# AdamQLMeng/PPNet

Hardware: AMD Instinct MI355X
Metric: edage_pp_map_path_instances_per_sec (higher is better)
Workload: dtype f64

## Files before the change

include/ppnet_hip.h:

```cpp
#ifndef PPNET_HIP_H
#define PPNET_HIP_H

#include <stdint.h>

#ifdef __cplusplus
extern "C" {
#endif

#define PPN_OK             0
#define PPN_E_INVALID     -1
#define PPN_E_HIP         -2
#define PPN_E_UNSUPPORTED -3

#define PPN_SEGS            10
#define PPN_POLY             5
#define PPN_PATH_POINTS   1000
#define PPN_BOUNDARY_POINTS 1100
#define PPN_DRAWS_PER_SEG 1002
#define PPN_DRAWS_PER_PATH (1 + PPN_SEGS * PPN_DRAWS_PER_SEG)
#define PPN_MAX_HULL        64
#define PPN_MAX_ISLES       16
#define PPN_MAX_POCKET      64
#define PPN_POCKET_TRY_CAP 256
#define PPN_PLACE_TRY_CAP 4096
// ... 304 lines not shown
                    const uint32_t* params , void* img_out ,
                    uint8_t* label_out , int B, int H, int W, int Ho, int Wo,
                    const float* mean3, const float* std3, int seg_pad_val, int dtype , void* stream);
int ppn_seg_labels_2class(const void* logits, uint8_t* labels, int32_t B, int32_t h, int32_t w, int32_t Ho, int32_t Wo,
                          int32_t dtype, void* stream);
int ppn_bias_act_nhwc(void* x, const void* bias, int64_t n, int32_t C, float negative_slope, int32_t dtype, void* stream);

int ppn_conv3x3_c1_nhwc(const void* x, const float* w, const float* bias, void* y, int32_t B, int32_t H, int32_t W,
                        int32_t Cout, float negative_slope, int32_t dtype, void* stream);
int ppn_conv3x3_to1_nhwc(const void* x, const float* w, float bias, void* y, int32_t B, int32_t H, int32_t W, int32_t Cin,
                         int32_t dtype, void* stream);

int ppn_conv3x3_mfma_bf16(const void* x, const void* w, const float* bias, void* y, int32_t B, int32_t H, int32_t W, int32_t Cin,
                          int32_t Cout, int32_t stride, int32_t relu, void* stream);
int32_t ppn_conv3x3_relu_classify2_slots(int32_t Cout);
int ppn_conv3x3_relu_classify2_bf16(const void* x, const void* w, const float* bias, const float* w2, float* logits, float* partial, int32_t B,
                                    int32_t H, int32_t W, int32_t Cin, int32_t Cout, void* stream);
int ppn_gennet_conv_s2_bf16(const void* x, const void* w, const float* bias, void* y, int32_t B, int32_t H, int32_t W, float negative_slope,
                            int32_t transposed, void* stream);
int ppn_gennet_dec_final_bf16(const void* x, const void* w, const float* bias, float negative_slope, const float* w_final, float bias_final, void* y,
                              int32_t B, int32_t H, int32_t W, void* stream);
int ppn_gennet_first_enc_bf16(const void* x1, const void* w1, const float* b1, const void* wk2, const float* bias2, void* y, int32_t B, int32_t H, int32_t W,
                              float slope1, float slope2, void* stream);
#define PPN_GENNET_BLOCK_PARAMS 7224
int ppn_gennet_trunk_bf16(const void* x, void* y, const float* params, int32_t B, int32_t N, int32_t n_blocks, void* stream);
int ppn_assemble_paths(const double* wp, const int32_t* wp_n, const uint8_t* ok, const double* init, const double* end, double rate, int32_t n,
                       int32_t max_wp, double* full, int32_t* counts, void* stream);
int ppn_plan_collision(const double* waypoints, const int32_t* counts, const void* obstacles, int32_t obstacles_f64, const int32_t* n_obstacles,
                       int32_t B, int32_t M, int32_t S, float clearance, float bound, uint8_t* collision, void* stream);
int ppn_heatmap_u8(const void* y, uint8_t* out, int32_t B, int32_t n, int32_t dtype, void* stream);
int ppn_tokenizer_conv1_codes_bf16(const uint8_t* grid, const void* lut, void* out, int32_t B, int32_t H, int32_t W, void* stream);
int ppn_tokenizer_codes_bf16(const uint8_t* grid, const void* lut, const void* w2p, const float* vec, void* tokens, int32_t B, int32_t H, int32_t W,
                             float eps, void* stream);
int ppn_nat128_ln_qkv_bf16(const void* s, const float* offset, const void* ln_w, const void* ln_b, const void* w, const void* bias, void* qkv,
                           int64_t tokens, float eps, void* stream);
int ppn_nat128_ln_mlp_bf16(void* s, const float* offset, const void* ln_w, const void* ln_b, const void* w1, const void* b1, const void* w2,
                           int64_t tokens, float eps, void* stream);
int ppn_nat128_ln_mlp_add_bf16(void* s, const float* offset, const void* ln_w, const void* ln_b, const void* w1, const void* b1, const void* w2,
                               const float* final_add, int64_t tokens, float eps, void* stream);
int ppn_nat128_proj_add_bf16(void* s, const void* a, const void* w, int64_t tokens, void* stream);

int ppn_gemm_bf16(const void* a, const void* w, const float* bias, void* c, int64_t M, int32_t N, int32_t K, int32_t epilogue,
                  int32_t persistent_blocks, void* stream);

int32_t ppn_nat_gemm_partials(int32_t C);

// ... 21 lines not shown
```

ppnet_amd/_lib.py:

```python
import ctypes as C
import os

_HERE = os.path.dirname(os.path.abspath(__file__))
LIB_PATH = os.environ.get("PPNET_HIP_LIB") or os.path.join(_HERE, "libppnet_hip.so")

PPN_OK = 0
PPN_E_UNSUPPORTED = -3
SEGS = 10
PATH_POINTS = 1000
BOUNDARY_POINTS = 1100
DRAWS_PER_SEG = 1002
DRAWS_PER_PATH = 1 + SEGS * DRAWS_PER_SEG
MAX_HULL = 64
MAX_ISLES = 16
MAX_POCKET = 64
POCKET_TRY_CAP = 256
PLACE_TRY_CAP = 4096
MAX_WAYPOINTS = 2048
GRID_OBST, GRID_FREE, GRID_MARK = 0, 255, 128
FLAG_POCKET_CAP, FLAG_PLACE_CAP, FLAG_EMPTY_ISLE, FLAG_HULL_CAP, FLAG_ISLE_CAP, FLAG_POCKET_FULL = 1, 2, 4, 8, 16, 32
FLAG_CORRIDOR_PASS = 64
FLAG_POCKET_DRAWS = 128

_p = C.c_void_p
# ... 19 lines not shown

ABI_VERSION = 111

EXPORTS = ("ppn_version", "ppn_error_string", "ppn_last_hip_error", "ppn_polyfit_table", "ppn_edage_paths",
           "ppn_edage_paths_ex", "ppn_edage_paths_ex2", "ppn_edage_maps", "ppn_edage_maps_place", "ppn_edage_maps_raster",
           "ppn_label_masks", "ppn_boundary_check", "ppn_boundary_check_ex",
           "ppn_obstacle_filter", "ppn_paint_markers", "ppn_disc_raster", "ppn_collision_segments", "ppn_collision_segments_bound",
           "ppn_extract_paths", "ppn_resize_bilinear_u8", "ppn_philox_doubles", "ppn_na2d_fwd", "ppn_na2d_fwd_padded", "ppn_na2d_fwd_vpad", "ppn_swin_wmsa_fwd", "ppn_swin_wmsa_bwd", "ppn_swin_wmsa_bwd_workspace", "ppn_mhsa_fwd", "ppn_mhsa_bwd", "ppn_mhsa_bwd_workspace", "ppn_na2d_bwd", "ppn_na2d_bwd_workspace", "ppn_na2d_bwd_vpad", "ppn_na2d_bwd_vpad_workspace", "ppn_residual_layernorm", "ppn_residual_layernorm_padded", "ppn_layernorm_offset", "ppn_upsample2x_nhwc", "ppn_resize_concat4_nhwc", "ppn_resize_concat_nhwc", "ppn_adaptive_pools_nhwc", "ppn_upsample2x_add_nhwc", "ppn_upsample2x_nhwc_bias", "ppn_upsample2x_concat_nhwc", "ppn_bias_act_nhwc", "ppn_seg_labels_2class", "ppn_grid_to_image", "ppn_conv3x3_c1_nhwc", "ppn_conv3x3_to1_nhwc",
           "ppn_conv3x3_mfma_bf16", "ppn_conv3x3_relu_classify2_bf16", "ppn_conv3x3_relu_classify2_slots", "ppn_gemm_bf16", "ppn_nat_gemm_bf16", "ppn_nat_gemm_partials", "ppn_row_stats_bf16", "ppn_nat_mlp_supported", "ppn_nat_mlp_pack_bf16", "ppn_nat_mlp_bf16", "ppn_gennet_conv_s2_bf16", "ppn_gennet_trunk_bf16",
           "ppn_assemble_paths", "ppn_plan_collision", "ppn_gennet_first_enc_bf16", "ppn_gennet_dec_final_bf16", "ppn_heatmap_u8", "ppn_tokenizer_conv1_codes_bf16", "ppn_tokenizer_codes_bf16", "ppn_nat128_ln_qkv_bf16", "ppn_nat128_ln_mlp_bf16", "ppn_nat128_ln_mlp_add_bf16", "ppn_nat128_proj_add_bf16",
           "ppn_resize_ce_workspace", "ppn_resize_ce_fwd", "ppn_resize_ce_bwd", "ppn_seg_eval",
           "ppn_augment_params", "ppn_augment_codes", "ppn_augment_rgb",
           "ppn_ohem_ce_workspace", "ppn_ohem_ce_fwd", "ppn_ohem_ce_bwd",
           "ppn_resize_dice_workspace", "ppn_resize_dice_fwd", "ppn_resize_dice_bwd",
           "ppn_upsample2x_nhwc_bwd", "ppn_upsample2x_concat_nhwc_bwd", "ppn_resize_concat_nhwc_bwd",
           "ppn_residual_layernorm_train_fwd", "ppn_residual_layernorm_bwd_workspace", "ppn_residual_layernorm_bwd",
           "ppn_patch_merge_ln_fwd", "ppn_patch_merge_ln_bwd_workspace", "ppn_patch_merge_ln_bwd", "ppn_patch_merge_ln_rows",
           "ppn_patch_merge_ln_max_blocks", "ppn_seg_tta",
           "ppn_gennet_stem_train_workspace", "ppn_gennet_stem_train_fwd", "ppn_gennet_stem_train_bwd", "ppn_gennet_stem_train_tile",
           "ppn_gennet_stem_train_max_blocks",
           "ppn_gennet_tail_train_workspace", "ppn_gennet_tail_train_fwd", "ppn_gennet_tail_train_bwd", "ppn_gennet_tail_train_tile",
           "ppn_gennet_tail_train_max_blocks",
           "ppn_gennet_s2_tile", "ppn_gennet_s2_max_blocks", "ppn_gennet_s2_wgrad_workspace", "ppn_gennet_s2_down", "ppn_gennet_s2_up",
           "ppn_gennet_s2_wgrad", "ppn_wmsa_fwd")


def _load():
    if not os.path.exists(LIB_PATH):
        raise ImportError(
            f"{LIB_PATH} is missing: the HIP extension is the only implementation of this package "
            f"(no CPU fallback). Build it with `python -c 'import __graft_entry__ as g; g.build()'` "
            f"or `make -C ppnet_amd/csrc`.")
    lib = C.CDLL(LIB_PATH)
    lib.ppn_version.restype = C.c_int
    if lib.ppn_version() != ABI_VERSION:
        raise ImportError(
            f"{LIB_PATH} reports ABI version {lib.ppn_version()}, these bindings are written against {ABI_VERSION} "
            f"(include/ppnet_hip.h: PPN_ABI_VERSION): argument lists differ, rebuild with `make -C ppnet_amd/csrc`.")
    lib.ppn_error_string.restype = C.c_char_p
    lib.ppn_error_string.argtypes = [C.c_int]
    lib.ppn_last_hip_error.restype = C.c_int
    lib.ppn_polyfit_table.argtypes = [_p]
    lib.ppn_edage_paths.argtypes = [C.c_int32, C.c_uint64, C.c_int32, C.c_double, C.c_double, C.c_uint64,
                                    _p, _p, C.c_int32, C.POINTER(PathsStruct), _p]
    lib.ppn_edage_paths_ex.argtypes = [C.c_int32, C.c_uint64, C.c_int32, C.c_double, C.c_double, C.c_uint64,
                                       _p, _p, C.c_int32, _p, C.POINTER(PathsStruct), _p]
    lib.ppn_edage_paths_ex2.argtypes = [C.c_int32, C.c_uint64, C.c_int32, C.c_double, C.c_double, C.c_uint64,
# ... 75 lines not shown
    lib.ppn_gennet_tail_train_bwd.argtypes = [_p] * 12 + [C.c_int] * 4 + [C.c_float, C.c_int, _p]
    lib.ppn_gennet_tail_train_tile.argtypes = []
    lib.ppn_gennet_tail_train_max_blocks.argtypes = []
    lib.ppn_gennet_s2_tile.argtypes = []
    lib.ppn_gennet_s2_max_blocks.argtypes = []
    lib.ppn_gennet_s2_wgrad_workspace.argtypes = [C.c_int] * 3
    lib.ppn_gennet_s2_wgrad_workspace.restype = C.c_int64
    lib.ppn_gennet_s2_down.argtypes = [_p] * 4 + [C.c_int] * 5 + [_p]
    lib.ppn_gennet_s2_up.argtypes = [_p] * 4 + [C.c_int] * 5 + [_p]
    lib.ppn_gennet_s2_wgrad.argtypes = [_p] * 6 + [C.c_int] * 5 + [_p]
    lib.ppn_grid_to_image.argtypes = [_p, _p, C.c_int64, C.POINTER(C.c_float), C.POINTER(C.c_float), C.c_int32, _p]
    lib.ppn_seg_labels_2class.argtypes = [_p, _p, C.c_int32, C.c_int32, C.c_int32, C.c_int32, C.c_int32, C.c_int32, _p]
    lib.ppn_bias_act_nhwc.argtypes = [_p, _p, C.c_int64, C.c_int32, C.c_float, C.c_int32, _p]
    lib.ppn_conv3x3_c1_nhwc.argtypes = [_p, _p, _p, _p, C.c_int32, C.c_int32, C.c_int32, C.c_int32, C.c_float, C.c_int32, _p]
    lib.ppn_conv3x3_to1_nhwc.argtypes = [_p, _p, C.c_float, _p, C.c_int32, C.c_int32, C.c_int32, C.c_int32, C.c_int32, _p]
    lib.ppn_conv3x3_mfma_bf16.argtypes = [_p, _p, _p, _p, C.c_int32, C.c_int32, C.c_int32, C.c_int32, C.c_int32, C.c_int32, C.c_int32, _p]
    lib.ppn_conv3x3_relu_classify2_bf16.argtypes = [_p, _p, _p, _p, _p, _p, C.c_int32, C.c_int32, C.c_int32, C.c_int32, C.c_int32, _p]
    lib.ppn_conv3x3_relu_classify2_slots.argtypes = [C.c_int32]
    lib.ppn_gennet_conv_s2_bf16.argtypes = [_p, _p, _p, _p, C.c_int32, C.c_int32, C.c_int32, C.c_float, C.c_int32, _p]
    lib.ppn_gennet_trunk_bf16.argtypes = [_p, _p, _p, C.c_int32, C.c_int32, C.c_int32, _p]
    lib.ppn_assemble_paths.argtypes = [_p, _p, _p, _p, _p, C.c_double, C.c_int32, C.c_int32, _p, _p, _p]
    lib.ppn_plan_collision.argtypes = [_p, _p, _p, C.c_int32, _p, C.c_int32, C.c_int32, C.c_int32, C.c_float, C.c_float, _p, _p]
    lib.ppn_gennet_first_enc_bf16.argtypes = [_p, _p, _p, _p, _p, _p, C.c_int32, C.c_int32, C.c_int32, C.c_float, C.c_float, _p]
    lib.ppn_gennet_dec_final_bf16.argtypes = [_p, _p, _p, C.c_float, _p, C.c_float, _p, C.c_int32, C.c_int32, C.c_int32, _p]
    lib.ppn_heatmap_u8.argtypes = [_p, _p, C.c_int32, C.c_int32, C.c_int32, _p]
    lib.ppn_tokenizer_conv1_codes_bf16.argtypes = [_p, _p, _p, C.c_int32, C.c_int32, C.c_int32, _p]
    lib.ppn_tokenizer_codes_bf16.argtypes = [_p, _p, _p, _p, _p, C.c_int32, C.c_int32, C.c_int32, C.c_float, _p]
    lib.ppn_nat128_ln_qkv_bf16.argtypes = [_p, _p, _p, _p, _p, _p, _p, C.c_int64, C.c_float, _p]
    lib.ppn_nat128_ln_mlp_bf16.argtypes = [_p, _p, _p, _p, _p, _p, _p, C.c_int64, C.c_float, _p]
    lib.ppn_nat128_ln_mlp_add_bf16.argtypes = [_p, _p, _p, _p, _p, _p, _p, _p, C.c_int64, C.c_float, _p]
    lib.ppn_nat128_proj_add_bf16.argtypes = [_p, _p, _p, C.c_int64, _p]
    lib.ppn_gemm_bf16.argtypes = [_p, _p, _p, _p, C.c_int64, C.c_int32, C.c_int32, C.c_int32, C.c_int32, _p]
    lib.ppn_nat_gemm_bf16.argtypes = [_p, _p, _p, _p, _p, C.c_int32, _p, _p, C.c_int64, C.c_int32, C.c_int32, C.c_int32, C.c_float, _p]
    lib.ppn_row_stats_bf16.argtypes = [_p, C.c_int64, C.c_int32, _p, _p]
    lib.ppn_nat_gemm_partials.argtypes = [C.c_int32]
    lib.ppn_nat_mlp_supported.argtypes = [C.c_int64, C.c_int32, C.c_int32]
    lib.ppn_nat_mlp_pack_bf16.argtypes = [_p, _p, _p, C.c_int32, C.c_int32, _p]
    lib.ppn_nat_mlp_bf16.argtypes = [_p, _p, _p, _p, _p, C.c_int64, C.c_int32, C.c_int32, C.c_float, _p]
    lib.ppn_resize_ce_workspace.argtypes = [C.c_int] * 3
    lib.ppn_resize_ce_workspace.restype = C.c_int64
    lib.ppn_resize_ce_fwd.argtypes = [_p, _p, _p, _p, _p, _p, C.c_int64] + [C.c_int] * 9 + [_p]
    lib.ppn_resize_ce_bwd.argtypes = [_p, _p, _p, _p, _p] + [C.c_int] * 9 + [_p]
    lib.ppn_seg_eval.argtypes = [_p, _p, _p, _p] + [C.c_int] * 9 + [_p]
    lib.ppn_seg_tta.argtypes = [C.POINTER(TtaAug), C.c_int, _p, _p] + [C.c_int] * 5 + [_p]
    lib.ppn_ohem_ce_workspace.argtypes = [C.c_int] * 3
    lib.ppn_ohem_ce_workspace.restype = C.c_int64
# ... 37 lines not shown
```

ppnet_amd/csrc/capi.hip:

```cpp
#include <hip/hip_runtime.h>
#include <math.h>
#include <mutex>
#include <stdlib.h>
#include <string.h>
#include <vector>

#include <cstdlib>
#include "ppn_kernels.h"

namespace {

thread_local int g_last_hip = 0;

inline int hip_fail(hipError_t e) {
    g_last_hip = (int)e;
    return PPN_E_HIP;
}
#define PPN_HIP(call) do { hipError_t e_ = (call); if (e_ != hipSuccess) return hip_fail(e_); } while (0)

inline bool bad_R(int R) { return R < 32 || R > 512 || (R % 32) != 0; }

void build_polyfit_table(double* out) {
    const int N = PPN_PATH_POINTS, M = 5;
    std::vector<long double> q((size_t)M * N);
// ... 1132 lines not shown
    const int e = ppn::conv3x3_mfma_launch(x, w, bias, nullptr, B, H, W, Cin, Cout, 1, 1, w2, logits, partial, (hipStream_t)stream);
    if (e != 0) return hip_fail((hipError_t)e);
    return PPN_OK;
}

int ppn_gennet_conv_s2_bf16(const void* x, const void* w, const float* bias, void* y, int32_t B, int32_t H, int32_t W, float negative_slope,
                            int32_t transposed, void* stream) {
    if (!x || !w || !bias || !y || B <= 0 || H <= 0 || W <= 0 || (!transposed && ((H | W) & 1))) return PPN_E_INVALID;
    if ((long long)B * H * W * 4 >= (1LL << 31)) return PPN_E_UNSUPPORTED;
    const int e = transposed ? ppn::gennet_dec_conv_launch(x, w, bias, y, B, H, W, negative_slope, (hipStream_t)stream)
                             : ppn::gennet_enc_conv_launch(x, w, bias, y, B, H, W, negative_slope, (hipStream_t)stream);
    if (e != 0) return hip_fail((hipError_t)e);
    return PPN_OK;
}

int ppn_gennet_first_enc_bf16(const void* x1, const void* w1, const float* b1, const void* wk2, const float* bias2, void* y, int32_t B, int32_t H, int32_t W,
                              float slope1, float slope2, void* stream) {
    if (!x1 || !w1 || !b1 || !wk2 || !bias2 || !y || B <= 0 || H <= 0 || W <= 0 || ((H | W) & 1)) return PPN_E_INVALID;
    const int e = ppn::gennet_first_enc_launch(x1, w1, b1, wk2, bias2, y, B, H, W, slope1, slope2, (hipStream_t)stream);
    if (e != 0) return hip_fail((hipError_t)e);
    return PPN_OK;
}

int ppn_gennet_dec_final_bf16(const void* x, const void* w, const float* bias, float negative_slope, const float* w_final, float bias_final, void* y,
                              int32_t B, int32_t H, int32_t W, void* stream) {
    if (!x || !w || !bias || !w_final || !y || B <= 0 || H <= 0 || W <= 0) return PPN_E_INVALID;
    if ((long long)B * H * W * 4 * 24 >= (1LL << 32)) return PPN_E_UNSUPPORTED;
    const int e = ppn::gennet_dec_final_launch(x, w, bias, negative_slope, w_final, bias_final, y, B, H, W, (hipStream_t)stream);
    if (e != 0) return hip_fail((hipError_t)e);
    return PPN_OK;
}

int ppn_gennet_trunk_bf16(const void* x, void* y, const float* params, int32_t B, int32_t N, int32_t n_blocks, void* stream) {
    if (!x || !y || !params || B <= 0 || N <= 0 || N > 1024 || (N % 8) != 0 || n_blocks <= 0) return PPN_E_INVALID;
    const int e = ppn::gennet_trunk_launch(x, y, params, B, N, n_blocks, (hipStream_t)stream);
    if (e != 0) return hip_fail((hipError_t)e);
    return PPN_OK;
}

int ppn_assemble_paths(const double* wp, const int32_t* wp_n, const uint8_t* ok, const double* init, const double* end, double rate, int32_t n,
                       int32_t max_wp, double* full, int32_t* counts, void* stream) {
    if (!wp || !wp_n || !ok || !init || !end || !full || !counts || n <= 0 || max_wp <= 0) return PPN_E_INVALID;
    const int e = ppn::assemble_paths_launch(wp, wp_n, ok, init, end, rate, n, max_wp, full, counts, (hipStream_t)stream);
    if (e != 0) return hip_fail((hipError_t)e);
    return PPN_OK;
}
// ... 155 lines not shown
```

ppnet_amd/csrc/gennet_conv.hip:

```cpp
#include <hip/hip_runtime.h>
#include "ppn_device.h"
#include "ppn_kernels.h"

namespace ppn {

namespace {
typedef __attribute__((ext_vector_type(8))) __bf16 bf16x8;
typedef __attribute__((ext_vector_type(4))) __bf16 bf16x4;
typedef __attribute__((ext_vector_type(4))) float f32x4;

__device__ __forceinline__ bf16x8 ld8(const __bf16* p) { return *reinterpret_cast<const bf16x8*>(p); }
__device__ __forceinline__ bf16x8 zero8() { return bf16x8{0, 0, 0, 0, 0, 0, 0, 0}; }

__device__ __forceinline__ void store4(__bf16* dst, const f32x4 v, const float4 b, float slope) {
    float o[4] = {v[0] + b.x, v[1] + b.y, v[2] + b.z, v[3] + b.w};
#pragma unroll
    for (int r = 0; r < 4; ++r) o[r] = o[r] > 0.f ? o[r] : o[r] * slope;
    *reinterpret_cast<bf16x4*>(dst) = bf16x4{(__bf16)o[0], (__bf16)o[1], (__bf16)o[2], (__bf16)o[3]};
}
__device__ __forceinline__ void store8(__bf16* dst, const f32x4 a0, const f32x4 a1, const float4 b0, const float4 b1, float slope) {
    float o[8] = {a0[0] + b0.x, a0[1] + b0.y, a0[2] + b0.z, a0[3] + b0.w, a1[0] + b1.x, a1[1] + b1.y, a1[2] + b1.z, a1[3] + b1.w};
#pragma unroll
    for (int r = 0; r < 8; ++r) o[r] = o[r] > 0.f ? o[r] : o[r] * slope;
    *reinterpret_cast<bf16x8*>(dst) = bf16x8{(__bf16)o[0], (__bf16)o[1], (__bf16)o[2], (__bf16)o[3], (__bf16)o[4], (__bf16)o[5], (__bf16)o[6], (__bf16)o[7]};
// ... 245 lines not shown
            const u32x4_ fw = {odd ? (w8 | 0x3F800000u) : e0, odd ? 0u : e1, odd ? 0u : e2, odd ? 0u : e3};
            const bf16x8 bw = __builtin_bit_cast(bf16x8, fw);
            f32x4 y0 = __builtin_amdgcn_mfma_f32_16x16x32_bf16(wa1[0], bw, f32x4{0.f, 0.f, 0.f, 0.f}, 0, 0, 0);
            f32x4 y1 = __builtin_amdgcn_mfma_f32_16x16x32_bf16(wa1[1], bw, f32x4{0.f, 0.f, 0.f, 0.f}, 0, 0, 0);
            const int py = 2 * oy + ty - 1, px = 2 * ox + tx - 1;
            const bool inside = py >= 0 && py < H && px >= 0 && px < W;
            float v[8] = {y0[0], y0[1], y0[2], y0[3], y1[0], y1[1], y1[2], y1[3]};
#pragma unroll
            for (int e = 0; e < 8; ++e) v[e] = fmaxf(v[e], v[e] * slope1);
            u32x4_ fv = {pack_bf16x2(v[0], v[1]), pack_bf16x2(v[2], v[3]), pack_bf16x2(v[4], v[5]), pack_bf16x2(v[6], v[7])};
            if (!inside) fv = u32x4_{0u, 0u, 0u, 0u};
            const bf16x8 fb = __builtin_bit_cast(bf16x8, fv);
            a0 = __builtin_amdgcn_mfma_f32_16x16x32_bf16(wa2[0][t], fb, a0, 0, 0, 0);
            a1 = __builtin_amdgcn_mfma_f32_16x16x32_bf16(wa2[1][t], fb, a1, 0, 0, 0);
        }
        if (live) {
            __bf16* dst = y + (size_t)pix * GC;
            store4(dst + 4 * g, a0, d0, slope2);
            if (g < 2) store4(dst + 16 + 4 * g, a1, d1, slope2);
        }
    }
}

int gennet_first_enc_launch(const void* x1, const void* w1, const float* b1, const void* wk2, const float* bias2, void* y, int B, int H, int W, float slope1,
                            float slope2, hipStream_t stream) {
    const long long total = (long long)B * (H / 2) * (W / 2);
    if ((long long)B * H * W >= (1LL << 31)) return (int)hipErrorInvalidValue;
    long long blocks = (total + 63) / 64;
    if (blocks > 256 * 12) blocks = 256 * 12;
    hipLaunchKernelGGL(gennet_first_enc_kernel, dim3((unsigned)blocks), dim3(256), 0, stream, (const __bf16*)x1, (const __bf16*)w1, b1,
                       (const __bf16*)wk2, bias2, (__bf16*)y, B, H, W, slope1, slope2);
    return (int)hipGetLastError();
}

int gennet_enc_conv_launch(const void* x, const void* wk, const float* bias, void* y, int B, int H, int W, float slope, hipStream_t stream) {
    const long long total = (long long)B * (H / 2) * (W / 2);
    long long blocks = (total + 16 * GROUPS * 4 - 1) / (16 * GROUPS * 4);
    if (blocks > 256 * 16) blocks = 256 * 16;
    hipLaunchKernelGGL(gennet_enc_conv_kernel, dim3((unsigned)blocks), dim3(256), 0, stream, (const __bf16*)x, (const __bf16*)wk, bias,
                       (__bf16*)y, B, H, W, slope);
    return (int)hipGetLastError();
}

int gennet_dec_final_launch(const void* x, const void* wt, const float* bias, float slope, const float* w1, float bias1, void* y, int B, int H, int W,
                            hipStream_t stream) {
    const long long tiles = (long long)B * ((2 * H + DF_H - 1) / DF_H) * ((2 * W + DF_W - 1) / DF_W);
// ... 20 lines not shown
```

ppnet_amd/csrc/ppn_kernels.h:

```cpp
#pragma once
#include <hip/hip_runtime.h>
#include <stdint.h>
#include <atomic>
#include "../../include/ppnet_hip.h"

#ifndef PPN_PATHS_THREADS
#define PPN_PATHS_THREADS 256
#endif

namespace ppn {

constexpr int PPN_MAX_DEVICES = 64;
inline int current_device() {
    int d = 0;
    return (hipGetDevice(&d) == hipSuccess && d >= 0 && d < PPN_MAX_DEVICES) ? d : -1;
}
struct DeviceOnce { std::atomic<int> done[PPN_MAX_DEVICES]; };
struct DeviceBuffer { std::atomic<void*> p[PPN_MAX_DEVICES]; };
inline int dynamic_lds_once(DeviceOnce& o, const void* fn, int bytes) {
    const int d = current_device();
    if (d < 0) return (int)hipErrorInvalidDevice;
    if (o.done[d].load(std::memory_order_acquire)) return 0;
    const hipError_t e = hipFuncSetAttribute(fn, hipFuncAttributeMaxDynamicSharedMemorySize, bytes);
    if (e != hipSuccess) return (int)e;
// ... 199 lines not shown
                       int label_dtype, hipStream_t stream);
int resize_dice_pixels();
int resize_dice_threads();
int resize_dice_max_classes();
long long resize_dice_workspace_bytes(int B, int C, int H, int W);
int resize_dice_fwd_launch(const void* logit, const void* label, const float* class_weight, void* workspace, float* lse, double* sums, float* loss,
                           int64_t* correct, int B, int C, int h, int w, int H, int W, int ignore_index, float smooth, int logit_dtype,
                           int label_dtype, hipStream_t stream);
int resize_dice_bwd_launch(const void* logit, const void* label, const float* lse, const double* sums, const float* class_weight,
                           const float* grad_out, void* workspace, void* dlogit, int B, int C, int h, int w, int H, int W, int ignore_index,
                           float smooth, int logit_dtype, int label_dtype, hipStream_t stream);
int augment_threads();
int augment_pixels();
int augment_params_launch(uint64_t seed, uint64_t first_instance, int B, double flip_ratio, double brightness_delta, double contrast_lo,
                          double contrast_hi, double saturation_lo, double saturation_hi, int hue_delta, uint32_t* params, hipStream_t stream);
int augment_launch(int rgb, const uint8_t* in, const uint8_t* label_in, const uint32_t* params, void* img, uint8_t* label_out, int B, int H, int W,
                   int Ho, int Wo, const float* mean, const float* stdv, int seg_pad_val, int dtype, hipStream_t stream);
int na2d_dense7_launch(const void* qkv, const void* pad_kv, const float* rpb, void* out, int B, int H, int W, int Hr, int Wr, int heads, int dil,
                       float scale, hipStream_t stream);
int gennet_dec_final_launch(const void* x, const void* wt, const float* bias, float slope, const float* w1, float bias1, void* y, int B, int H, int W,
                            hipStream_t stream);
int gennet_first_enc_launch(const void* x1, const void* w1, const float* b1, const void* wk2, const float* bias2, void* y, int B, int H, int W, float slope1,
                            float slope2, hipStream_t stream);
int heatmap_u8_launch(const void* y, uint8_t* out, int B, int n, int dtype, hipStream_t stream);
int tokenizer_fused_launch(const uint8_t* grid, const void* lut, const void* w2p, const float* vec, void* out, int B, int H, int W, float eps,
                           hipStream_t stream);
int tokenizer_codes_launch(const uint8_t* grid, const void* lut, void* out, int B, int H, int W, hipStream_t stream);
int nat128_ln_qkv_launch(const void* s, const float* off, const void* lnw, const void* lnb, const void* w, const void* bias, void* qkv, long long tokens,
                         float eps, hipStream_t stream);
int nat128_ln_mlp_launch(void* s, const float* off, const void* lnw, const void* lnb, const void* w1, const void* b1, const void* w2, const float* add,
                         long long tokens, float eps, hipStream_t stream);
int nat128_proj_add_launch(void* s, const void* a, const void* w, long long tokens, hipStream_t stream);
int gennet_trunk_launch(const void* x, void* y, const float* params, int B, int N, int n_blocks, hipStream_t stream);
bool gemm_small_wanted(long long M, int N, int K);
int gemm_small_launch(const void* a, const void* w, const float* bias, void* c, long long M, int N, int K, int epilogue, hipStream_t stream);
bool nat_mlp_supported(long long M, int C, int HID);
int nat_mlp_pack_launch(const void* w1, const void* w2, void* wpk, int C, int HID, hipStream_t stream);
int nat_mlp_launch(void* s, const void* wpk, const float* hb, const float* b2, float* stats_out, long long M, int C, int HID, float eps, hipStream_t stream);
bool nat_stats_p128(int C);
int row_stats_launch(const void* x, long long rows, int C, float* stats, hipStream_t stream);
int gemm_acc_stats_launch(const void* a, const void* w, const float* bias, float* stats, void* c, long long M, int N, int K, int n_cu,
                          hipStream_t stream);
int gemm_ln_launch(const void* a, const void* w, const float* bias, const float* colsum, const float* stats, int parts, void* c, long long M,
                   int N, int K, int gelu, float eps, int n_cu, hipStream_t stream);
int gemm_mfma_launch(const void* a, const void* w, const float* bias, void* c, long long M, int N, int K, int epi, int persistent,
                     hipStream_t stream);
// ... 6 lines not shown
```

ppnet_amd/fused.py:

```python
import ctypes
import os

import torch
import torch.nn.functional as F
from torch.autograd.function import once_differentiable

from . import _lib as L

_DT = {torch.float32: 0, torch.bfloat16: 1}


def _p(t):
    return ctypes.c_void_p(t.data_ptr()) if t is not None else ctypes.c_void_p(None)


class WeightCache:
    __slots__ = ("key", "value", "__weakref__")
    _all = None

    def __init__(self):
        self.key = self.value = None
        if WeightCache._all is None:
            import weakref
            WeightCache._all = weakref.WeakSet()
# ... 835 lines not shown
    y = torch.empty(B, 1, 2 * H, 2 * W, dtype=x.dtype, device=x.device)
    with torch.cuda.device(x.device):
        rc = L.lib.ppn_gennet_dec_final_bf16(_p(x), _p(w_packed), _p(bias32), float(negative_slope), _p(w_final32), float(bias_final), _p(y), B, H, W,
                                             ctypes.c_void_p(torch.cuda.current_stream(x.device).cuda_stream))
    L.check(rc, "ppn_gennet_dec_final_bf16")
    return y


def gennet_first_enc(x, w1, b1, wk2, b2, slope1, slope2):
    if not x.is_cuda or x.dtype != torch.bfloat16:
        raise RuntimeError("ppnet_amd.fused.gennet_first_enc: bfloat16 GPU tensors only")
    B, _, H, W = x.shape
    x = x.contiguous()
    assert w1.shape == (2, 16, 32) and wk2.shape == (2, 9, 16, 32) and w1.dtype == wk2.dtype == torch.bfloat16
    assert b1.dtype == b2.dtype == torch.float32 and b1.numel() == b2.numel() == 32
    y = torch.empty(B, H // 2, W // 2, 24, dtype=x.dtype, device=x.device)
    with torch.cuda.device(x.device):
        rc = L.lib.ppn_gennet_first_enc_bf16(_p(x), _p(w1), _p(b1), _p(wk2), _p(b2), _p(y), B, H, W, float(slope1), float(slope2),
                                             ctypes.c_void_p(torch.cuda.current_stream(x.device).cuda_stream))
    L.check(rc, "ppn_gennet_first_enc_bf16")
    return y.permute(0, 3, 1, 2)


def gennet_trunk(x_nchw_cl, params32, n_blocks):
    if not x_nchw_cl.is_cuda or x_nchw_cl.dtype != torch.bfloat16:
        raise RuntimeError("ppnet_amd.fused.gennet_trunk: bfloat16 GPU tensors only")
    x = x_nchw_cl.permute(0, 2, 3, 1)
    if not x.is_contiguous():
        x = x.contiguous()
    B, H, W, C = x.shape
    assert C == 24 and params32.dtype == torch.float32 and params32.is_contiguous() and params32.numel() == n_blocks * 7224
    y = torch.empty_like(x)
    with torch.cuda.device(x.device):
        rc = L.lib.ppn_gennet_trunk_bf16(_p(x), _p(y), _p(params32), B, H * W, n_blocks,
                                         ctypes.c_void_p(torch.cuda.current_stream(x.device).cuda_stream))
    L.check(rc, "ppn_gennet_trunk_bf16")
    return y.permute(0, 3, 1, 2)


LOSS_CALLS = {"fwd": 0, "bwd": 0}
_LABEL_DT = {torch.uint8: 0, torch.int64: 1}
_INT32_END = 1 << 31
RESIZE_CE_THREADS = 256
RESIZE_CE_FWD_PIXELS = 1024


# ... 790 lines not shown
```

ppnet_amd/gennet.py:

```python
import math
from functools import partial

import os

import torch
import torch.nn as nn
import torch.nn.functional as F

from . import fused
from . import swin
from .dense import drop_path, gpu_inference, linear
from .vit import mhsa_autograd


class _Attention(nn.Module):
    def __init__(self, dim, num_heads, qkv_bias=True):
        super().__init__()
        self.num_heads = num_heads
        self.scale = (dim // num_heads) ** -0.5
        self.qkv = nn.Linear(dim, dim * 3, bias=qkv_bias)
        self.proj = nn.Linear(dim, dim)

    def forward(self, x):
        B, N, C = x.shape
# ... 155 lines not shown
        dpr = [float(v) for v in torch.linspace(0, 0.1, 3)]
        self.vit_blocks = nn.Sequential(*[_Block(dim, 3, 4, dpr[i]) for i in range(3)])
        self.dec_conv = nn.ModuleList(_stage(nn.ConvTranspose2d(dim, dim, 3, 2, 1, output_padding=1)) for _ in range(n_down))
        self.conv_final = nn.Conv2d(dim, out_channels, 3, 1, 1)
        self._final_f32 = None
        self._trunk = fused.WeightCache()
        self._first_enc = fused.WeightCache()

    def prepare_inference(self):
        for stage in [self.conv_first, *self.enc_conv, *self.dec_conv]:
            _fold_bn(stage)
        self.to(memory_format=torch.channels_last)
        self.conv_first = _FusedStage(self.conv_first[0], self.conv_first[2].negative_slope)
        self.enc_conv = nn.ModuleList(_FusedStage(st[0], st[2].negative_slope) for st in self.enc_conv)
        self.dec_conv = nn.ModuleList(_FusedStage(st[0], st[2].negative_slope) for st in self.dec_conv)
        self._final_f32 = fused.WeightCache()
        return self

    def _final_pack(self):
        cf = self.conv_final
        return self._final_f32.get((cf.weight, cf.bias), lambda: (
            cf.weight.detach().float().contiguous(), float(cf.bias.detach().float()[0]) if cf.bias is not None and cf.out_channels == 1 else 0.0))

    def _fused_first_stage(self, x):
        cf = self.conv_first
        if not (isinstance(cf, _FusedStage) and len(self.enc_conv) > 0 and isinstance(self.enc_conv[0], _FusedStage) and x.is_cuda
                and x.dtype == torch.bfloat16 and not os.environ.get("PPNET_GENNET_UNFUSED")):
            return None
        c1, c2 = cf.conv, self.enc_conv[0].conv
        if not (isinstance(c1, nn.Conv2d) and c1.in_channels == 1 and c1.out_channels == 24 and c1.kernel_size == (3, 3) and c1.stride == (1, 1)
                and c1.padding == (1, 1) and c1.bias is not None and isinstance(c2, nn.Conv2d) and _is_s2_stage(c2)
                and x.shape[-1] % 2 == 0 and x.shape[-2] % 2 == 0):
            return None
        packs = self._first_enc.get((c1.weight, c1.bias, c2.weight, c2.bias), lambda: pack_first_enc_weights(c1, c2))
        return fused.gennet_first_enc(x, *packs, cf.slope, self.enc_conv[0].slope)

    def forward(self, x):
        y = self._fused_first_stage(x)
        if y is not None:
            x = y
            for blk in self.enc_conv[1:]:
                x = blk(x)
        else:
            cf = self.conv_first
            if (isinstance(cf, nn.Sequential) and len(cf) == 3 and type(cf[2]) is nn.LeakyReLU and fused.stem_train_ok(x, cf[0], cf[1])):
                x = fused.stem_bn_act(x, cf[0], cf[1], cf[2].negative_slope)
            else:
                x = cf(x)
            for blk in self.enc_conv:
                x = _run_stage(blk, x)
        B, C, H, W = x.shape
        if (x.is_cuda and x.dtype == torch.bfloat16 and self._final_f32 is not None and C == 24 and H * W <= 1024 and (H * W) % 8 == 0
                and self.vit_blocks[0].attn.num_heads == 3 and not os.environ.get("PPNET_LIBRARY_TRUNK")):
            trunk = self._trunk.get(list(self.vit_blocks.parameters()), lambda: pack_trunk_params(self.vit_blocks).to(x.device))
            x = fused.gennet_trunk(x.contiguous(memory_format=torch.channels_last), trunk, len(self.vit_blocks))
        else:
            t = self.vit_blocks(x.flatten(2).transpose(1, 2))
            x = t.transpose(1, 2).reshape(B, C, H, W)
        c = self.conv_final
        last = self.dec_conv[-1] if len(self.dec_conv) else None
        if (isinstance(last, _FusedStage) and x.is_cuda and x.dtype == torch.bfloat16 and self._final_f32 is not None and c.out_channels == 1
# ... 292 lines not shown
```

ppnet_amd/ppnet.py:

```python
import os

import torch

from . import _lib as L
from . import edage, plan
from .gennet import AEViT, normalize_heatmap_u8
from .segnet import SegNet, normalize_images


_TUNED = os.environ.get("PPNET_TUNED_TABLE") or os.path.join(os.path.dirname(os.path.abspath(__file__)), "tuned_gemm_gfx950_b256.csv")


def _use_tuned_gemms():
    try:
        import torch.cuda.tunable as tn
        if os.path.exists(_TUNED) and torch.cuda.is_available():
            import tempfile
            tn.enable(True)
            retune = os.environ.get("PPNET_TUNE_GEMMS")
            tn.tuning_enable(bool(retune))
            tn.set_filename(retune or os.path.join(tempfile.gettempdir(), f"ppnet_amd_tunableop_{os.getpid()}.csv"))
            tn.read_file(_TUNED)
    except Exception as e:
        import sys
# ... 27 lines not shown
            self.gennet.to(weights_dtype)

    @torch.no_grad()
    def segment(self, grid_u8):
        rgb = edage.grid_to_rgb(grid_u8) * 255.0
        x = normalize_images(rgb)
        if self.weights_dtype is not None:
            x = x.to(self.weights_dtype)
        with torch.autocast("cuda", dtype=self.amp_dtype, enabled=self.amp_dtype is not None):
            return self.segnet(x)

    @torch.no_grad()
    def segment_u8(self, grid_u8):
        from .segnet import IMG_MEAN, IMG_STD
        from . import fused
        if self.amp_dtype is None and self.segnet.backbone.patch_embed.takes_codes(grid_u8):
            return self.segnet.labels_u8(grid_u8)
        x = fused.grid_to_image(grid_u8, IMG_MEAN, IMG_STD, self.weights_dtype or torch.float32)
        with torch.autocast("cuda", dtype=self.amp_dtype, enabled=self.amp_dtype is not None):
            return self.segnet.labels_u8(x)

    @torch.no_grad()
    def heatmap(self, mask):
        x = mask.to(self.weights_dtype or torch.float32).unsqueeze(1)
        with torch.autocast("cuda", dtype=self.amp_dtype, enabled=self.amp_dtype is not None):
            y = self.gennet(x)
        from . import fused
        return fused.heatmap_u8(y) if y.is_cuda else normalize_heatmap_u8(y)

    @torch.no_grad()
    def plan(self, grid_u8, init, end, obstacles, n_obstacles, clearance=None, down_sample_rate=2):
        heat = self.heatmap(self.segment(grid_u8) if os.environ.get("PPNET_NO_FUSED_TAIL") else self.segment_u8(grid_u8))
        return self.plan_tail(heat, init, end, obstacles, n_obstacles, clearance, down_sample_rate)

    @torch.no_grad()
    def generate_and_plan(self, paths, maps, placements, first_path_id=0, first_map_id=0, seed=0, obstacles_size=5, obstacles_num=20,
                          clearance=None, down_sample_rate=2, mark=None, gennet_input="segnet"):
        mark = mark or (lambda name: None)
        mark("start")
        edage.generate_paths(paths.n, paths.R, paths.map_size, paths.clearance, seed=seed, first_path_id=first_path_id,
                             device=paths.device, out=paths)
        edage.generate_maps(paths, placements, obstacles_size, obstacles_num, seed=seed, first_map_id=first_map_id, out=maps)
        mark("generated")
        mask = self.segment_u8(maps.grid)
        mark("segmented")
        if gennet_input == "labels":
            _, space = edage.label_masks(paths, maps, placements, want_path=False, want_space=True)
            heat = self.heatmap(space)
        else:
            heat = self.heatmap(mask)
# ... 45 lines not shown
```

Before: 54.80 million.

## Feed binary masks directly into GenNet first stage via precomputed conv table

Adds a kernel that takes the uint8 segmentation mask directly and skips the cast to a bf16 image. Because the input is binary, the first 3x3 conv plus LeakyReLU output depends only on a 9-bit neighbourhood pattern. The kernel precomputes all 512 outputs into shared memory with MFMA, then runs the stride-2 conv by table lookup on bit-packed mask rows. This removes the float conversion pass and the first conv's arithmetic and memory traffic, at the cost of more code complexity. It also adds an atomic counter that records any mask values other than 0 or 1.

```diff
diff --git a/include/ppnet_hip.h b/include/ppnet_hip.h
--- a/include/ppnet_hip.h
+++ b/include/ppnet_hip.h
@@ -350,6 +350,8 @@
                               int32_t B, int32_t H, int32_t W, void* stream);
 int ppn_gennet_first_enc_bf16(const void* x1, const void* w1, const float* b1, const void* wk2, const float* bias2, void* y, int32_t B, int32_t H, int32_t W,
                               float slope1, float slope2, void* stream);
+int ppn_gennet_first_enc_labels_bf16(const uint8_t* mask, const void* w1, const float* b1, const void* wk2, const float* bias2, void* y, int32_t B, int32_t H,
+                                     int32_t W, float slope1, float slope2, int32_t* violations, void* stream);
 #define PPN_GENNET_BLOCK_PARAMS 7224
 int ppn_gennet_trunk_bf16(const void* x, void* y, const float* params, int32_t B, int32_t N, int32_t n_blocks, void* stream);
 int ppn_assemble_paths(const double* wp, const int32_t* wp_n, const uint8_t* ok, const double* init, const double* end, double rate, int32_t n,
diff --git a/ppnet_amd/_lib.py b/ppnet_amd/_lib.py
--- a/ppnet_amd/_lib.py
+++ b/ppnet_amd/_lib.py
@@ -65,7 +65,7 @@
            "ppn_gennet_tail_train_workspace", "ppn_gennet_tail_train_fwd", "ppn_gennet_tail_train_bwd", "ppn_gennet_tail_train_tile",
            "ppn_gennet_tail_train_max_blocks",
            "ppn_gennet_s2_tile", "ppn_gennet_s2_max_blocks", "ppn_gennet_s2_wgrad_workspace", "ppn_gennet_s2_down", "ppn_gennet_s2_up",
-           "ppn_gennet_s2_wgrad", "ppn_wmsa_fwd")
+           "ppn_gennet_s2_wgrad", "ppn_wmsa_fwd", "ppn_gennet_first_enc_labels_bf16")
 
 
 def _load():
@@ -187,6 +187,7 @@
     lib.ppn_assemble_paths.argtypes = [_p, _p, _p, _p, _p, C.c_double, C.c_int32, C.c_int32, _p, _p, _p]
     lib.ppn_plan_collision.argtypes = [_p, _p, _p, C.c_int32, _p, C.c_int32, C.c_int32, C.c_int32, C.c_float, C.c_float, _p, _p]
     lib.ppn_gennet_first_enc_bf16.argtypes = [_p, _p, _p, _p, _p, _p, C.c_int32, C.c_int32, C.c_int32, C.c_float, C.c_float, _p]
+    lib.ppn_gennet_first_enc_labels_bf16.argtypes = [_p, _p, _p, _p, _p, _p, C.c_int32, C.c_int32, C.c_int32, C.c_float, C.c_float, _p, _p]
     lib.ppn_gennet_dec_final_bf16.argtypes = [_p, _p, _p, C.c_float, _p, C.c_float, _p, C.c_int32, C.c_int32, C.c_int32, _p]
     lib.ppn_heatmap_u8.argtypes = [_p, _p, C.c_int32, C.c_int32, C.c_int32, _p]
     lib.ppn_tokenizer_conv1_codes_bf16.argtypes = [_p, _p, _p, C.c_int32, C.c_int32, C.c_int32, _p]
diff --git a/ppnet_amd/csrc/capi.hip b/ppnet_amd/csrc/capi.hip
--- a/ppnet_amd/csrc/capi.hip
+++ b/ppnet_amd/csrc/capi.hip
@@ -1178,6 +1178,16 @@
     return PPN_OK;
 }
 
+int ppn_gennet_first_enc_labels_bf16(const uint8_t* mask, const void* w1, const float* b1, const void* wk2, const float* bias2, void* y, int32_t B, int32_t H,
+                                     int32_t W, float slope1, float slope2, int32_t* violations, void* stream) {
+    if (!mask || !w1 || !b1 || !wk2 || !bias2 || !y || B <= 0 || H < 2 || W < 2 || ((H | W) & 1) || !(slope1 <= 1.0f)) return PPN_E_INVALID;
+    if (reinterpret_cast<uintptr_t>(mask) & 1) return PPN_E_INVALID;
+    if ((long long)B * H * W >= (1LL << 31)) return PPN_E_UNSUPPORTED;
+    const int e = ppn::gennet_first_enc_labels_launch(mask, w1, wk2, bias2, y, B, H, W, slope1, slope2, violations, (hipStream_t)stream);
+    if (e != 0) return hip_fail((hipError_t)e);
+    return PPN_OK;
+}
+
 int ppn_gennet_dec_final_bf16(const void* x, const void* w, const float* bias, float negative_slope, const float* w_final, float bias_final, void* y,
                               int32_t B, int32_t H, int32_t W, void* stream) {
     if (!x || !w || !bias || !w_final || !y || B <= 0 || H <= 0 || W <= 0) return PPN_E_INVALID;
diff --git a/ppnet_amd/csrc/gennet_conv.hip b/ppnet_amd/csrc/gennet_conv.hip
--- a/ppnet_amd/csrc/gennet_conv.hip
+++ b/ppnet_amd/csrc/gennet_conv.hip
@@ -291,6 +291,112 @@
     }
 }
 
+namespace {
+constexpr int FT_ZERO = 512;
+
+__device__ __forceinline__ uint32_t mask_row_bits(const uint8_t* __restrict__ mb, int iy, int c, int H, int W, bool& bad) {
+    const int cy = min(max(iy, 0), H - 1);
+    uint32_t u[3];
+#pragma unroll
+    for (int k = 0; k < 3; ++k) {
+        const int cx = min(max(c + 2 * k, 0), W - 2);
+        u[k] = *reinterpret_cast<const uint16_t*>(mb + (uint32_t)(cy * W + cx));
+    }
+    u[2] &= 0xffu;
+    bad = ((u[0] | u[1] | u[2]) & 0xfefeu) != 0u;
+    return (u[0] & 1u) | ((u[0] >> 7) & 2u) | ((u[1] & 1u) << 2) | ((u[1] >> 5) & 8u) | ((u[2] & 1u) << 4);
+}
+}
+
+__global__ __launch_bounds__(256, 4) void gennet_first_enc_labels_kernel(const uint8_t* __restrict__ mask, const __bf16* __restrict__ w1,
+                                                                      const __bf16* __restrict__ wk2, const float* __restrict__ bias2,
+                                                                      __bf16* __restrict__ y, int B, int H, int W, float slope1, float slope2,
+                                                                      int* __restrict__ violations) {
+    typedef __attribute__((ext_vector_type(4))) uint32_t u32x4_;
+    __shared__ u32x4_ T[(FT_ZERO + 1) * 4];
+    const int lane = threadIdx.x & 63, pl = lane & 15, g = lane >> 4;
+    {
+        bf16x8 wa1[2];
+#pragma unroll
+        for (int nt = 0; nt < 2; ++nt) wa1[nt] = ld8(w1 + (nt * 16 + pl) * 32 + g * 8);
+        const bool odd = g & 1;
+        for (int cg = (threadIdx.x >> 6) * 8; cg < (threadIdx.x >> 6) * 8 + 8; ++cg) {
+            const uint32_t p = cg * 16 + pl;
+            auto val2 = [&](int i0, int i1) -> uint32_t { return ((p >> i0) & 1u) * 0x3F80u | ((p >> i1) & 1u) * 0x3F800000u; };
+            const uint32_t e0 = val2(0, 1), e1 = val2(2, 3), e2 = val2(4, 5), e3 = val2(6, 7);
+            const uint32_t w8 = ((p >> 8) & 1u) * 0x3F80u;
+            const u32x4_ fw = {odd ? (w8 | 0x3F800000u) : e0, odd ? 0u : e1, odd ? 0u : e2, odd ? 0u : e3};
+            const bf16x8 bw = __builtin_bit_cast(bf16x8, fw);
+            f32x4 y0 = __builtin_amdgcn_mfma_f32_16x16x32_bf16(wa1[0], bw, f32x4{0.f, 0.f, 0.f, 0.f}, 0, 0, 0);
+            f32x4 y1 = __builtin_amdgcn_mfma_f32_16x16x32_bf16(wa1[1], bw, f32x4{0.f, 0.f, 0.f, 0.f}, 0, 0, 0);
+            float v[8] = {y0[0], y0[1], y0[2], y0[3], y1[0], y1[1], y1[2], y1[3]};
+#pragma unroll
+            for (int e = 0; e < 8; ++e) v[e] = fmaxf(v[e], v[e] * slope1);
+            T[p * 4 + g] = u32x4_{pack_bf16x2(v[0], v[1]), pack_bf16x2(v[2], v[3]), pack_bf16x2(v[4], v[5]), pack_bf16x2(v[6], v[7])};
+        }
+        if (threadIdx.x < 4) T[FT_ZERO * 4 + threadIdx.x] = u32x4_{0u, 0u, 0u, 0u};
+    }
+    __syncthreads();
+    const int Ho = H >> 1, Wo = W >> 1;
+    bf16x8 wa2[2][9];
+#pragma unroll
+    for (int nt = 0; nt < 2; ++nt)
+#pragma unroll
+        for (int t = 0; t < 9; ++t) wa2[nt][t] = ld8(wk2 + ((nt * 9 + t) * 16 + pl) * 32 + g * 8);
+    const float4 d0 = *reinterpret_cast<const float4*>(bias2 + 4 * g), d1 = *reinterpret_cast<const float4*>(bias2 + 16 + 4 * g);
+    const uint32_t total32 = (uint32_t)B * Ho * Wo, wave = blockIdx.x * 4 + (threadIdx.x >> 6), nwaves = gridDim.x * 4;
+    const uint32_t per_img = (uint32_t)Wo * Ho;
+    for (uint32_t base = wave * 16; base < total32; base += nwaves * 16) {
+        uint32_t pix = base + pl;
+        const bool live = pix < total32;
+        if (!live) pix = total32 - 1;
+        const uint32_t img = pix / per_img, rem = pix - img * per_img;
+        const int oy = (int)(rem / (uint32_t)Wo), ox = (int)(rem - (uint32_t)oy * Wo);
+        const uint8_t* mb = mask + (size_t)img * H * W;
+        bool bad_g, bad_4;
+        uint32_t bits = mask_row_bits(mb, 2 * oy - 2 + g, 2 * ox - 2, H, W, bad_g) << (5 * g);
+        const uint32_t row4 = mask_row_bits(mb, 2 * oy + 2, 2 * ox - 2, H, W, bad_4) << 20;
+        if ((live & (bad_g | (bad_4 & (g == 0)))) && violations) atomicAdd(violations, 1);
+        bits |= __shfl_xor((int)bits, 16);
+        bits |= __shfl_xor((int)bits, 32);
+        bits |= row4;
+        uint32_t valid = 0x1FFFFFFu;
+        valid &= oy == 0 ? ~0x3FFu : ~0u;
+        valid &= oy == Ho - 1 ? ~0x1F00000u : ~0u;
+        valid &= ox == 0 ? ~0x318C63u : ~0u;
+        valid &= ox == Wo - 1 ? ~0x1084210u : ~0u;
+        bits &= valid;
+        f32x4 a0 = {0.f, 0.f, 0.f, 0.f}, a1 = a0;
+#pragma unroll
+        for (int t = 0; t < 9; ++t) {
+            const int ty = t / 3, tx = t % 3;
+            uint32_t p = ((bits >> (5 * ty + tx)) & 7u) | (((bits >> (5 * ty + 5 + tx)) & 7u) << 3) | (((bits >> (5 * ty + 10 + tx)) & 7u) << 6);
+            if (ty == 0 && tx == 0) p = (oy == 0 || ox == 0) ? FT_ZERO : p;
+            else if (ty == 0) p = oy == 0 ? FT_ZERO : p;
+            else if (tx == 0) p = ox == 0 ? FT_ZERO : p;
+            const bf16x8 fb = __builtin_bit_cast(bf16x8, T[p * 4 + g]);
+            a0 = __builtin_amdgcn_mfma_f32_16x16x32_bf16(wa2[0][t], fb, a0, 0, 0, 0);
+            a1 = __builtin_amdgcn_mfma_f32_16x16x32_bf16(wa2[1][t], fb, a1, 0, 0, 0);
+        }
+        if (live) {
+            __bf16* dst = y + (size_t)pix * GC;
+            store4(dst + 4 * g, a0, d0, slope2);
+            if (g < 2) store4(dst + 16 + 4 * g, a1, d1, slope2);
+        }
+    }
+}
+
+int gennet_first_enc_labels_launch(const uint8_t* mask, const void* w1, const void* wk2, const float* bias2, void* y, int B, int H, int W, float slope1,
+                                   float slope2, int* violations, hipStream_t stream) {
+    const long long total = (long long)B * (H / 2) * (W / 2);
+    if ((long long)B * H * W >= (1LL << 31)) return (int)hipErrorInvalidValue;
+    long long blocks = (total + 63) / 64;
+    if (blocks > 256 * 12) blocks = 256 * 12;
+    hipLaunchKernelGGL(gennet_first_enc_labels_kernel, dim3((unsigned)blocks), dim3(256), 0, stream, mask, (const __bf16*)w1, (const __bf16*)wk2, bias2,
+                       (__bf16*)y, B, H, W, slope1, slope2, violations);
+    return (int)hipGetLastError();
+}
+
 int gennet_first_enc_launch(const void* x1, const void* w1, const float* b1, const void* wk2, const float* bias2, void* y, int B, int H, int W, float slope1,
                             float slope2, hipStream_t stream) {
     const long long total = (long long)B * (H / 2) * (W / 2);
diff --git a/ppnet_amd/csrc/ppn_kernels.h b/ppnet_amd/csrc/ppn_kernels.h
--- a/ppnet_amd/csrc/ppn_kernels.h
+++ b/ppnet_amd/csrc/ppn_kernels.h
@@ -245,6 +245,8 @@
                             hipStream_t stream);
 int gennet_first_enc_launch(const void* x1, const void* w1, const float* b1, const void* wk2, const float* bias2, void* y, int B, int H, int W, float slope1,
                             float slope2, hipStream_t stream);
+int gennet_first_enc_labels_launch(const uint8_t* mask, const void* w1, const void* wk2, const float* bias2, void* y, int B, int H, int W, float slope1,
+                                   float slope2, int* violations, hipStream_t stream);
 int heatmap_u8_launch(const void* y, uint8_t* out, int B, int n, int dtype, hipStream_t stream);
 int tokenizer_fused_launch(const uint8_t* grid, const void* lut, const void* w2p, const float* vec, void* out, int B, int H, int W, float eps,
                            hipStream_t stream);
diff --git a/ppnet_amd/fused.py b/ppnet_amd/fused.py
--- a/ppnet_amd/fused.py
+++ b/ppnet_amd/fused.py
@@ -881,6 +881,47 @@
     return y.permute(0, 3, 1, 2)
 
 
+_LABEL_VIOLATIONS = {}
+
+
+def _label_violation_word(device):
+    device = torch.device("cuda", torch.cuda.current_device()) if device.index is None else device
+    w = _LABEL_VIOLATIONS.get(device)
+    if w is None:
+        w = _LABEL_VIOLATIONS[device] = torch.zeros(1, dtype=torch.int32, device=device)
+    return w
+
+
+def gennet_label_violations(device):
+    w = _label_violation_word(torch.device(device))
+    n = int(w.item())
+    w.zero_()
+    return n
+
+
+def gennet_first_enc_labels(mask, w1, b1, wk2, b2, slope1, slope2):
+    if not mask.is_cuda or mask.dtype not in (torch.uint8, torch.bool):
+        raise RuntimeError("ppnet_amd.fused.gennet_first_enc_labels: uint8 / bool GPU masks only")
+    if mask.dim() == 4:
+        assert mask.shape[1] == 1
+        mask = mask[:, 0]
+    B, H, W = mask.shape
+    mask = mask.contiguous()
+    if mask.dtype == torch.bool:
+        mask = mask.view(torch.uint8)
+    if mask.data_ptr() & 1:
+        mask = mask.clone()
+    assert w1.shape == (2, 16, 32) and wk2.shape == (2, 9, 16, 32) and w1.dtype == wk2.dtype == torch.bfloat16
+    assert b1.dtype == b2.dtype == torch.float32 and b1.numel() == b2.numel() == 32
+    word = _label_violation_word(mask.device)
+    y = torch.empty(B, H // 2, W // 2, 24, dtype=torch.bfloat16, device=mask.device)
+    with torch.cuda.device(mask.device):
+        rc = L.lib.ppn_gennet_first_enc_labels_bf16(_p(mask), _p(w1), _p(b1), _p(wk2), _p(b2), _p(y), B, H, W, float(slope1), float(slope2), _p(word),
+                                                    ctypes.c_void_p(torch.cuda.current_stream(mask.device).cuda_stream))
+    L.check(rc, "ppn_gennet_first_enc_labels_bf16")
+    return y.permute(0, 3, 1, 2)
+
+
 def gennet_trunk(x_nchw_cl, params32, n_blocks):
     if not x_nchw_cl.is_cuda or x_nchw_cl.dtype != torch.bfloat16:
         raise RuntimeError("ppnet_amd.fused.gennet_trunk: bfloat16 GPU tensors only")
diff --git a/ppnet_amd/gennet.py b/ppnet_amd/gennet.py
--- a/ppnet_amd/gennet.py
+++ b/ppnet_amd/gennet.py
@@ -201,21 +201,40 @@
         return self._final_f32.get((cf.weight, cf.bias), lambda: (
             cf.weight.detach().float().contiguous(), float(cf.bias.detach().float()[0]) if cf.bias is not None and cf.out_channels == 1 else 0.0))
 
-    def _fused_first_stage(self, x):
+    def _first_stage_fuses(self, x, dtype):
         cf = self.conv_first
         if not (isinstance(cf, _FusedStage) and len(self.enc_conv) > 0 and isinstance(self.enc_conv[0], _FusedStage) and x.is_cuda
-                and x.dtype == torch.bfloat16 and not os.environ.get("PPNET_GENNET_UNFUSED")):
+                and dtype == torch.bfloat16 and not os.environ.get("PPNET_GENNET_UNFUSED")):
+            return False
+        c1, c2 = cf.conv, self.enc_conv[0].conv
+        return (isinstance(c1, nn.Conv2d) and c1.in_channels == 1 and c1.out_channels == 24 and c1.kernel_size == (3, 3) and c1.stride == (1, 1)
+                and c1.padding == (1, 1) and c1.bias is not None and isinstance(c2, nn.Conv2d) and _is_s2_stage(c2)
+                and x.shape[-1] % 2 == 0 and x.shape[-2] % 2 == 0)
+
+    def _first_packs(self):
+        c1, c2 = self.conv_first.conv, self.enc_conv[0].conv
+        return self._first_enc.get((c1.weight, c1.bias, c2.weight, c2.bias), lambda: pack_first_enc_weights(c1, c2))
+
+    def _fused_first_stage(self, x):
+        if not self._first_stage_fuses(x, x.dtype):
             return None
-        c1, c2 = cf.conv, self.enc_conv[0].conv
-        if not (isinstance(c1, nn.Conv2d) and c1.in_channels == 1 and c1.out_channels == 24 and c1.kernel_size == (3, 3) and c1.stride == (1, 1)
-                and c1.padding == (1, 1) and c1.bias is not None and isinstance(c2, nn.Conv2d) and _is_s2_stage(c2)
-                and x.shape[-1] % 2 == 0 and x.shape[-2] % 2 == 0):
-            return None
-        packs = self._first_enc.get((c1.weight, c1.bias, c2.weight, c2.bias), lambda: pack_first_enc_weights(c1, c2))
-        return fused.gennet_first_enc(x, *packs, cf.slope, self.enc_conv[0].slope)
-
-    def forward(self, x):
-        y = self._fused_first_stage(x)
+        return fused.gennet_first_enc(x, *self._first_packs(), self.conv_first.slope, self.enc_conv[0].slope)
+
+    def takes_labels(self, mask):
+        return (mask.dtype in (torch.uint8, torch.bool) and (mask.dim() == 3 or (mask.dim() == 4 and mask.shape[1] == 1))
+                and self._first_stage_fuses(mask, self.conv_final.weight.dtype) and mask.shape[-1] >= 2 and mask.shape[-2] >= 2
+                and self.conv_first.slope <= 1 and os.environ.get("PPNET_GENNET_FIRST_TABLE", "1") != "0")
+
+    def _fused_first_stage_labels(self, mask):
+        return fused.gennet_first_enc_labels(mask, *self._first_packs(), self.conv_first.slope, self.enc_conv[0].slope)
+
+    def forward(self, x):
+        if x.dtype in (torch.uint8, torch.bool):
+            if not self.takes_labels(x):
+                raise RuntimeError("AEViT.forward: this model does not take a class mask here (see takes_labels); pass the mask as a float image")
+            y = self._fused_first_stage_labels(x)
+        else:
+            y = self._fused_first_stage(x)
         if y is not None:
             x = y
             for blk in self.enc_conv[1:]:
diff --git a/ppnet_amd/ppnet.py b/ppnet_amd/ppnet.py
--- a/ppnet_amd/ppnet.py
+++ b/ppnet_amd/ppnet.py
@@ -73,10 +73,16 @@
 
     @torch.no_grad()
     def heatmap(self, mask):
-        x = mask.to(self.weights_dtype or torch.float32).unsqueeze(1)
-        with torch.autocast("cuda", dtype=self.amp_dtype, enabled=self.amp_dtype is not None):
-            y = self.gennet(x)
         from . import fused
+        takes = getattr(self.gennet, "takes_labels", None)
+        seg = getattr(getattr(self.segnet, "decode_head", None), "conv_seg", None)
+        binary = mask.dtype == torch.bool or (seg is not None and seg.out_channels <= 2)
+        if self.amp_dtype is None and self.weights_dtype == torch.bfloat16 and binary and takes is not None and takes(mask):
+            y = self.gennet(mask)
+        else:
+            x = mask.to(self.weights_dtype or torch.float32).unsqueeze(1)
+            with torch.autocast("cuda", dtype=self.amp_dtype, enabled=self.amp_dtype is not None):
+                y = self.gennet(x)
         return fused.heatmap_u8(y) if y.is_cuda else normalize_heatmap_u8(y)
 
     @torch.no_grad()
```

Measured after the change: 54.83 million (median of 3 runs). About the same (+0.0%).
